# GuanRunwei/ASY-VRNet

Hardware: AMD Instinct MI355X
Metric: images/sec fwd+bwd, 512x512 img+4ch radar, bs=8/GPU (higher is better)
Workload: dtype f32; 1 GPU; EfficientVRNet(phi=l) forward+backward, 512x512 image + 4x512x512 radar, bs=8/GPU, fp32, det+seg heads (BASELINE.json configs[1]); random weights; global_batch=8, image_size=512, parallelism=dp1, launch=hipgraph

## Files before the change

### asy-vrnet_amd/csrc/fusion.hip

```cpp
#include "common.h"

namespace {

__device__ __forceinline__ f32x4 ld4(const float* p) { return *reinterpret_cast<const f32x4*>(p); }
__device__ __forceinline__ float bn_pre(float A, float x, float S, float D) { return __builtin_fmaf(A, x - S, D); }

__device__ __forceinline__ void col_stats_flush(const double (&s1)[4], const double (&s2)[4], int CV, double* partial, double* lds) {
  const int tid = threadIdx.x;
#pragma unroll
  for (int j = 0; j < 4; ++j) {
    lds[tid * 8 + j] = s1[j];
    lds[tid * 8 + 4 + j] = s2[j];
  }
  __syncthreads();
  if (tid < CV) {
    const int off = (int)(((long)blockIdx.x * 256) % CV);
    int t0 = tid - off;
    if (t0 < 0) t0 += CV;
    double a[4] = {0, 0, 0, 0}, b[4] = {0, 0, 0, 0};
    for (int t = t0; t < 256; t += CV)
#pragma unroll
      for (int j = 0; j < 4; ++j) {
        a[j] += lds[t * 8 + j];
        b[j] += lds[t * 8 + 4 + j];
      }
    double* o = partial + ((long)blockIdx.x * CV + tid) * 8;
#pragma unroll
    for (int j = 0; j < 4; ++j) {
      o[2 * j] = a[j];
      o[2 * j + 1] = b[j];
    }
  }
}

__device__ __forceinline__ void minmax_fold(const float* partial, int nblocks, float* smn, float* smx, float& mn, float& mx) {
  mn = INFINITY;
  mx = -INFINITY;
  for (int e = threadIdx.x; e < nblocks; e += 256) {
    mn = fminf(mn, partial[2 * e]);
    mx = fmaxf(mx, partial[2 * e + 1]);
  }
#pragma unroll
  for (int o = 32; o > 0; o >>= 1) {
    mn = fminf(mn, __shfl_xor(mn, o, 64));
    mx = fmaxf(mx, __shfl_xor(mx, o, 64));
  }
  if ((threadIdx.x & 63) == 0) {
    smn[threadIdx.x >> 6] = mn;
    smx[threadIdx.x >> 6] = mx;
  }
  __syncthreads();
  mn = fminf(fminf(smn[0], smn[1]), fminf(smn[2], smn[3]));
  mx = fmaxf(fmaxf(smx[0], smx[1]), fmaxf(smx[2], smx[3]));
}

template <bool RES>
__global__ __launch_bounds__(256) void bn_relu_kernel(const float* __restrict__ z, const float* __restrict__ A, const float* __restrict__ D,
                                                      const float* __restrict__ S, const float* __restrict__ res, float* __restrict__ out,
                                                      long n4, int C, float* __restrict__ mmpart, double* __restrict__ colpart) {
  __shared__ double lds[RES ? 256 * 8 : 1];
  __shared__ float smn[4], smx[4];
  const int CV = C >> 2;
  const long G = (long)gridDim.x * 256, e0 = (long)blockIdx.x * 256 + threadIdx.x;
  const int c0 = (int)(e0 % CV) * 4;
  const f32x4 a4 = ld4(A + c0), d4 = ld4(D + c0), s4 = ld4(S + c0);
  double s1[4] = {0, 0, 0, 0}, s2[4] = {0, 0, 0, 0};
  float mn = INFINITY, mx = -INFINITY;
  for (long e = e0; e < n4; e += G) {
    const f32x4 zv = ld4(z + 4 * e);
    f32x4 r4 = {0.f, 0.f, 0.f, 0.f}, o;
    if (RES) r4 = ld4(res + 4 * e);
#pragma unroll
    for (int j = 0; j < 4; ++j) {
      float v = fmaxf(bn_pre(a4[j], zv[j], s4[j], d4[j]), 0.f);
      if (RES) {
        v += r4[j];
        s1[j] += (double)v;
        s2[j] += (double)v * (double)v;
      } else {
        mn = fminf(mn, v);
        mx = fmaxf(mx, v);
      }
      o[j] = v;
    }
    *reinterpret_cast<f32x4*>(out + 4 * e) = o;
  }
  if (RES) {
    col_stats_flush(s1, s2, CV, colpart, lds);
  } else {
#pragma unroll
    for (int o = 32; o > 0; o >>= 1) {
      mn = fminf(mn, __shfl_xor(mn, o, 64));
      mx = fmaxf(mx, __shfl_xor(mx, o, 64));
    }
    if ((threadIdx.x & 63) == 0) {
      smn[threadIdx.x >> 6] = mn;
      smx[threadIdx.x >> 6] = mx;
    }
    __syncthreads();
    if (threadIdx.x == 0) {
      mmpart[2 * blockIdx.x] = fminf(fminf(smn[0], smn[1]), fminf(smn[2], smn[3]));
      mmpart[2 * blockIdx.x + 1] = fmaxf(fmaxf(smx[0], smx[1]), fmaxf(smx[2], smx[3]));
    }
  }
}

__global__ __launch_bounds__(256) void enhance_stats_kernel(const float* p, const float* x, const float* mmpart, int nmm, float* mm,
                                                            float* t, long n4, int C, double* colpart) {
  __shared__ double lds[256 * 8];
  __shared__ float smn[4], smx[4];
  float mn, mx;
  minmax_fold(mmpart, nmm, smn, smx, mn, mx);
  if (blockIdx.x == 0 && threadIdx.x == 0) { mm[0] = mn; mm[1] = mx; }
  const float dst = mx - mn;
  const int CV = C >> 2;
  const long G = (long)gridDim.x * 256, e0 = (long)blockIdx.x * 256 + threadIdx.x;
  double s1[4] = {0, 0, 0, 0}, s2[4] = {0, 0, 0, 0};
  for (long e = e0; e < n4; e += G) {
    const f32x4 pv = ld4(p + 4 * e), xv = ld4(x + 4 * e);
    f32x4 o;
#pragma unroll
    for (int j = 0; j < 4; ++j) {
      o[j] = (1.f + (pv[j] - mn) / dst) * xv[j];
      s1[j] += (double)o[j];
      s2[j] += (double)o[j] * (double)o[j];
    }
    *reinterpret_cast<f32x4*>(t + 4 * e) = o;
  }
  col_stats_flush(s1, s2, CV, colpart, lds);
}

__global__ __launch_bounds__(256) void bn_bwd_enhance_kernel(const float* g, const float* t, const float* A, const float* E,
                                                             const float* D, const float* S, const float* x, const float* p,
                                                             const float* mm, float* dt, long n4, int C, double* sums4) {
  __shared__ double red[4][4];
  const int CV = C >> 2;
  const long G = (long)gridDim.x * 256, e0 = (long)blockIdx.x * 256 + threadIdx.x;
  const int c0 = (int)(e0 % CV) * 4;
  const f32x4 a4 = ld4(A + c0), e4 = ld4(E + c0), d4 = ld4(D + c0), s4 = ld4(S + c0);
  const float mn = mm[0], mx = mm[1];
  double s[4] = {0, 0, 0, 0};
  for (long e = e0; e < n4; e += G) {
    const f32x4 gv = ld4(g + 4 * e), tv = ld4(t + 4 * e), xv = ld4(x + 4 * e), pv = ld4(p + 4 * e);
    f32x4 o;
#pragma unroll
    for (int j = 0; j < 4; ++j) {
      float v = a4[j] * gv[j];
      v += e4[j] * (tv[j] - s4[j]);
      v += d4[j];
      o[j] = v;
      const double dn = (double)v * (double)xv[j];
      s[0] += dn;
      s[1] += dn * (double)(pv[j] - mn);
      s[2] += (pv[j] == mn) ? 1.0 : 0.0;
      s[3] += (pv[j] == mx) ? 1.0 : 0.0;
    }
    *reinterpret_cast<f32x4*>(dt + 4 * e) = o;
  }
#pragma unroll
  for (int i = 0; i < 4; ++i) s[i] = wave_sum(s[i]);
  if ((threadIdx.x & 63) == 0)
#pragma unroll
    for (int i = 0; i < 4; ++i) red[threadIdx.x >> 6][i] = s[i];
  __syncthreads();
  if (threadIdx.x < 4)
    sums4[4 * (long)blockIdx.x + threadIdx.x] = red[0][threadIdx.x] + red[1][threadIdx.x] + red[2][threadIdx.x] + red[3][threadIdx.x];
}

__global__ __launch_bounds__(256) void enhance_bwd_stats_kernel(const float* dt, const float* x, const float* p, const float* mm,
                                                                const double* sums4, int nsums, const float* z, const float* fA,
                                                                const float* fD, const float* fS, float* dx, float* dp, long n4,
                                                                int C, int accumulate_dx, double* colpart) {
  __shared__ double lds[256 * 8];
  __shared__ double red[4][4];
  __shared__ double sums[4];
  {
    double s[4] = {0, 0, 0, 0};
    for (int e = threadIdx.x; e < nsums; e += 256)
#pragma unroll
      for (int i = 0; i < 4; ++i) s[i] += sums4[4 * (long)e + i];
#pragma unroll
    for (int i = 0; i < 4; ++i) s[i] = wave_sum(s[i]);
    if ((threadIdx.x & 63) == 0)
#pragma unroll
      for (int i = 0; i < 4; ++i) red[threadIdx.x >> 6][i] = s[i];
    __syncthreads();
    if (threadIdx.x < 4) sums[threadIdx.x] = red[0][threadIdx.x] + red[1][threadIdx.x] + red[2][threadIdx.x] + red[3][threadIdx.x];
    __syncthreads();
  }
  const float mn = mm[0], mx = mm[1];
  const double dstd = (double)mx - (double)mn;
  const float gmn = (float)((-sums[0] / dstd + sums[1] / (dstd * dstd)) / sums[2]);
  const float gmx = (float)((-sums[1] / (dstd * dstd)) / sums[3]);
  const float fd = (float)dstd;
  const int CV = C >> 2;
  const long G = (long)gridDim.x * 256, e0 = (long)blockIdx.x * 256 + threadIdx.x;
  const int c0 = (int)(e0 % CV) * 4;
  const f32x4 a4 = ld4(fA + c0), d4 = ld4(fD + c0), s4 = ld4(fS + c0);
  double s1[4] = {0, 0, 0, 0}, s2[4] = {0, 0, 0, 0};
  for (long e = e0; e < n4; e += G) {
    const f32x4 gv = ld4(dt + 4 * e), xv = ld4(x + 4 * e), pv = ld4(p + 4 * e), zv = ld4(z + 4 * e);
    f32x4 ox, op;
    if (accumulate_dx) ox = ld4(dx + 4 * e);
#pragma unroll
    for (int j = 0; j < 4; ++j) {
      const float gain = 1.f + (pv[j] - mn) / fd;
      const float vx = gv[j] * gain;
      ox[j] = accumulate_dx ? ox[j] + vx : vx;
      float v = gv[j] * xv[j] / fd;
      if (pv[j] == mn) v += gmn;
      if (pv[j] == mx) v += gmx;
      op[j] = v;
      const float vm = (bn_pre(a4[j], zv[j], s4[j], d4[j]) > 0.f) ? v : 0.f;
      s1[j] += (double)vm;
      s2[j] += (double)vm * (double)zv[j];
    }
    *reinterpret_cast<f32x4*>(dx + 4 * e) = ox;
    *reinterpret_cast<f32x4*>(dp + 4 * e) = op;
  }
  col_stats_flush(s1, s2, CV, colpart, lds);
}

__global__ __launch_bounds__(256) void bn_bwd_next_stats_kernel(const float* __restrict__ g, const float* __restrict__ sx,
                                                                const float* __restrict__ A, const float* __restrict__ E,
                                                                const float* __restrict__ D, const float* __restrict__ S,
                                                                const float* __restrict__ z, const float* __restrict__ fA,
                                                                const float* __restrict__ fD, const float* __restrict__ fS,
                                                                float* __restrict__ ds, long n4, int C, double* __restrict__ colpart) {
  __shared__ double lds[256 * 8];
  const int CV = C >> 2;
  const long G = (long)gridDim.x * 256, e0 = (long)blockIdx.x * 256 + threadIdx.x;
  const int c0 = (int)(e0 % CV) * 4;
  const f32x4 a4 = ld4(A + c0), e4 = ld4(E + c0), d4 = ld4(D + c0), s4 = ld4(S + c0);
  const f32x4 fa4 = ld4(fA + c0), fd4 = ld4(fD + c0), fs4 = ld4(fS + c0);
  double s1[4] = {0, 0, 0, 0}, s2[4] = {0, 0, 0, 0};
  for (long e = e0; e < n4; e += G) {
    const f32x4 gv = ld4(g + 4 * e), xv = ld4(sx + 4 * e), zv = ld4(z + 4 * e);
    f32x4 o;
#pragma unroll
    for (int j = 0; j < 4; ++j) {
      float v = a4[j] * gv[j];
      v += e4[j] * (xv[j] - s4[j]);
      v += d4[j];
      o[j] = v;
      const float vm = (bn_pre(fa4[j], zv[j], fs4[j], fd4[j]) > 0.f) ? v : 0.f;
      s1[j] += (double)vm;
      s2[j] += (double)vm * (double)zv[j];
    }
    *reinterpret_cast<f32x4*>(ds + 4 * e) = o;
  }
  col_stats_flush(s1, s2, CV, colpart, lds);
}

int fusion_grid(long n4, int CV, long cap = 4096) {
  int g = 256, a = CV;
  while (a) { const int t = g % a; g = a; a = t; }
  const int m = CV / g;
  long nb = vr_cdiv(n4, 256 * 2);
  if (nb > cap) nb = cap;
  if (nb < 1) nb = 1;
  nb = vr_cdiv(nb, m) * m;
  return (int)nb;
}
bool fusion_ok(long n, int C) { return C % 4 == 0 && C >= 4 && C <= 1024 && n % C == 0 && n / 4 < (1L << 40); }
#define FUSION_ALIGNED(...)                                                        \
  [&] {                                                                            \
    const void* ps_[] = {__VA_ARGS__};                                             \
    for (const void* q_ : ps_)                                                     \
      if (q_ && !vr_aligned16(q_)) return false;                                   \
    return true;                                                                   \
  }()

}

extern "C" int vrnet_fusion_chunks(long n, int C) { return fusion_ok(n, C) ? fusion_grid(n / 4, C / 4) : 0; }
extern "C" int vrnet_fusion_fold_chunks(long n, int C) { return fusion_ok(n, C) ? fusion_grid(n / 4, C / 4, 1024) : 0; }

extern "C" int vrnet_bn_relu_minmax_f32(const float* z, const float* A, const float* D, const float* S, float* p, long n, int C,
                                        float* mmpart, void* stream) {
  VR_CHECK_ARG(z && A && D && S && p && mmpart && fusion_ok(n, C) && FUSION_ALIGNED(z, A, D, S, p), "bn_relu_minmax: bad arguments");
  if (vr_ablated("affine")) return VR_OK;
  hipLaunchKernelGGL((bn_relu_kernel<false>), dim3(fusion_grid(n / 4, C / 4, 1024)), dim3(256), 0, vr_stream(stream), z, A, D, S,
                     (const float*)nullptr, p, n / 4, C, mmpart, (double*)nullptr);
  VR_LAUNCH_CHECK("bn_relu_minmax");
  return VR_OK;
}

extern "C" int vrnet_bn_relu_res_stats_f32(const float* z, const float* A, const float* D, const float* S, const float* res,
                                           float* s, long n, int C, double* colpart, void* stream) {
  VR_CHECK_ARG(z && A && D && S && res && s && colpart && fusion_ok(n, C) && FUSION_ALIGNED(z, A, D, S, res, s),
               "bn_relu_res_stats: bad arguments");
  if (vr_ablated("affine")) return VR_OK;
  hipLaunchKernelGGL((bn_relu_kernel<true>), dim3(fusion_grid(n / 4, C / 4)), dim3(256), 0, vr_stream(stream), z, A, D, S, res, s,
                     n / 4, C, (float*)nullptr, colpart);
  VR_LAUNCH_CHECK("bn_relu_res_stats");
  return VR_OK;
}

extern "C" int vrnet_enhance_stats_f32(const float* p, const float* x, const float* mmpart, int nmm, float* mm, float* t, long n,
                                       int C, double* colpart, void* stream) {
  VR_CHECK_ARG(p && x && mmpart && nmm > 0 && mm && t && colpart && fusion_ok(n, C) && FUSION_ALIGNED(p, x, t),
               "enhance_stats: bad arguments");
  if (vr_ablated("misc")) return VR_OK;
  hipLaunchKernelGGL(enhance_stats_kernel, dim3(fusion_grid(n / 4, C / 4)), dim3(256), 0, vr_stream(stream), p, x, mmpart, nmm, mm,
                     t, n / 4, C, colpart);
  VR_LAUNCH_CHECK("enhance_stats");
  return VR_OK;
}

extern "C" int vrnet_bn_bwd_enhance_f32(const float* g, const float* t, const float* A, const float* E, const float* D,
                                        const float* S, const float* x, const float* p, const float* mm, float* dt, long n, int C,
                                        double* sums4, void* stream) {
  VR_CHECK_ARG(g && t && A && E && D && S && x && p && mm && dt && sums4 && fusion_ok(n, C) &&
                   FUSION_ALIGNED(g, t, A, E, D, S, x, p, dt), "bn_bwd_enhance: bad arguments");
  if (vr_ablated("affine")) return VR_OK;
  hipLaunchKernelGGL(bn_bwd_enhance_kernel, dim3(fusion_grid(n / 4, C / 4, 1024)), dim3(256), 0, vr_stream(stream), g, t, A, E, D, S, x, p,
                     mm, dt, n / 4, C, sums4);
  VR_LAUNCH_CHECK("bn_bwd_enhance");
  return VR_OK;
}

extern "C" int vrnet_enhance_bwd_stats_f32(const float* dt, const float* x, const float* p, const float* mm, const double* sums4,
                                           int nsums, const float* z, const float* fA, const float* fD, const float* fS, float* dx,
                                           float* dp, long n, int C, int accumulate_dx, double* colpart, void* stream) {
  VR_CHECK_ARG(dt && x && p && mm && sums4 && nsums > 0 && z && fA && fD && fS && dx && dp && colpart && fusion_ok(n, C) &&
                   FUSION_ALIGNED(dt, x, p, z, fA, fD, fS, dx, dp), "enhance_bwd_stats: bad arguments");
  if (vr_ablated("misc")) return VR_OK;
  hipLaunchKernelGGL(enhance_bwd_stats_kernel, dim3(fusion_grid(n / 4, C / 4)), dim3(256), 0, vr_stream(stream), dt, x, p, mm, sums4,
                     nsums, z, fA, fD, fS, dx, dp, n / 4, C, accumulate_dx, colpart);
  VR_LAUNCH_CHECK("enhance_bwd_stats");
  return VR_OK;
}

extern "C" int vrnet_bn_bwd_next_stats_f32(const float* g, const float* s, const float* A, const float* E, const float* D,
                                           const float* S, const float* z, const float* fA, const float* fD, const float* fS,
                                           float* ds, long n, int C, double* colpart, void* stream) {
  VR_CHECK_ARG(g && s && A && E && D && S && z && fA && fD && fS && ds && colpart && fusion_ok(n, C) &&
                   FUSION_ALIGNED(g, s, A, E, D, S, z, fA, fD, fS, ds), "bn_bwd_next_stats: bad arguments");
  if (vr_ablated("affine")) return VR_OK;
  hipLaunchKernelGGL(bn_bwd_next_stats_kernel, dim3(fusion_grid(n / 4, C / 4)), dim3(256), 0, vr_stream(stream), g, s, A, E, D, S, z,
                     fA, fD, fS, ds, n / 4, C, colpart);
  VR_LAUNCH_CHECK("bn_bwd_next_stats");
  return VR_OK;
}
```

### asy-vrnet_amd/csrc/spatial.hip

```cpp
#include "common.h"

#include <cstdlib>

namespace {

__global__ __launch_bounds__(256) void dwconv3x3_kernel(const float* x, long ldx, const float* w, float* y, long ldy,
                                                        int B, int H, int W, int C, int flip, int accumulate) {
  const int total = B * H * W * C;
  for (int e = blockIdx.x * 256 + threadIdx.x; e < total; e += gridDim.x * 256) {
    const int c = e % C;
    const int pix = e / C;
    const int xx = pix % W;
    const int q = pix / W;
    const int yy = q % H;
    const int b = q / H;
    float s = 0.f;
#pragma unroll
    for (int ky = 0; ky < 3; ++ky) {
      const int sy = yy + ky - 1;
      if (sy < 0 || sy >= H) continue;
      const float* row = x + ((long)(b * H + sy) * W) * ldx + c;
#pragma unroll
      for (int kx = 0; kx < 3; ++kx) {
        const int sx = xx + kx - 1;
// ... 213 lines not shown
#pragma unroll
    for (int t = 0; t < 9; ++t) *reinterpret_cast<f32x4*>(smx + (((rest - 1) * quads + cq) * 9 + t) * 4) = acc[t];
  }
  __syncthreads();
  if (rest == 0 && c < C) {
    for (int r = 1; r < groups; ++r)
#pragma unroll
      for (int t = 0; t < 9; ++t) acc[t] += *reinterpret_cast<const f32x4*>(smx + (((r - 1) * quads + cq) * 9 + t) * 4);
    float* d = partial + ((long)blockIdx.x * C + c) * 9;
#pragma unroll
    for (int j = 0; j < 4; ++j)
#pragma unroll
      for (int t = 0; t < 9; ++t) d[j * 9 + t] = acc[t][j];
  }
}
__global__ __launch_bounds__(256) void dwconv3x3_wgrad_reduce_kernel(const float* partial, int nchunks, int C, float* dw,
                                                                     int accumulate) {
  __shared__ double red[16][16];
  const int o = threadIdx.x & 15, sl = threadIdx.x >> 4;
  const int e = blockIdx.x * 16 + o;
  const bool live = e < C * 9;
  double s = 0;
  if (live)
    for (int k = sl; k < nchunks; k += 16) s += partial[(long)k * C * 9 + e];
  red[sl][o] = s;
  __syncthreads();
  if (sl == 0 && live) {
#pragma unroll
    for (int k = 1; k < 16; ++k) s += red[k][o];
    dw[e] = (accumulate ? dw[e] : 0.f) + (float)s;
  }
}

__global__ __launch_bounds__(256) void patch_gather_kernel(const float* x, long ldx, const float* pos, float* out, int B,
                                                           int H, int W, int C, int CP, int k) {
  const int CT = C + CP, KT = k * k * CT, OH = H / k, OW = W / k;
  const long total = (long)B * OH * OW * KT;
  for (long e = (long)blockIdx.x * 256 + threadIdx.x; e < total; e += (long)gridDim.x * 256) {
    const int ch = e % KT;
    const long op = e / KT;
    const int t = ch / CT, c = ch - t * CT;
    const int ky = t / k, kx = t - ky * k;
    const int ox = op % OW;
    const long q = op / OW;
    const int oy = q % OH;
    const long b = q / OH;
    const int yy = oy * k + ky, xx = ox * k + kx;
    out[e] = c < C ? x[((b * H + yy) * W + xx) * ldx + c] : pos[((long)yy * W + xx) * CP + (c - C)];
  }
}
__global__ __launch_bounds__(256) void patch_scatter_kernel(const float* dp, float* dx, long lddx, int B, int H, int W, int C,
                                                            int CP, int k, int accumulate) {
  const int CT = C + CP, KT = k * k * CT, OH = H / k, OW = W / k;
  const long total = (long)B * H * W * C;
  for (long e = (long)blockIdx.x * 256 + threadIdx.x; e < total; e += (long)gridDim.x * 256) {
    const int c = e % C;
    const long pix = e / C;
    const int xx = pix % W;
    const long q = pix / W;
    const int yy = q % H;
    const long b = q / H;
    const int t = (yy % k) * k + (xx % k);
    const float v = dp[((b * OH + yy / k) * OW + xx / k) * KT + t * CT + c];
    float* d = dx + pix * lddx + c;
    *d = accumulate ? *d + v : v;
  }
}
__global__ void ohwi_kernel(const float* src, float* dst, int Cout, int Cin, int T, int dir, int accumulate) {
  const long total = (long)Cout * Cin * T;
  const long e = (long)blockIdx.x * blockDim.x + threadIdx.x;
  if (e >= total) return;
  const int t = e % T;
  const long q = e / T;
  const int c = q % Cin;
  const long n = q / Cin;
  const long oihw = e, ohwi = (n * T + t) * Cin + c;
  if (dir == 0) dst[ohwi] = src[oihw];
  else dst[oihw] = (accumulate ? dst[oihw] : 0.f) + src[ohwi];
}

template <bool FUSED_L = false>
__device__ __forceinline__ void src_index(float scale, int o, int in_size, int* i0, int* i1, float* l1) {
#pragma clang fp contract(off)
  const float r = scale * (float)o;
  int a = (int)r;
  if (a > in_size - 1) a = in_size - 1;
  *i0 = a;
  *i1 = a + ((a < in_size - 1) ? 1 : 0);
  *l1 = FUSED_L ? __builtin_fmaf(scale, (float)o, -(float)a) : r - (float)a;
}

__device__ __forceinline__ float up_tap(float v, bool bn, float a, float d, float s) {
  return bn ? fmaxf(__builtin_fmaf(a, v - s, d), 0.f) : v;
}
__device__ __forceinline__ float up_tap(float v, const float* bnA, const float* bnD, const float* bnS, int c) {
  return bnA ? up_tap(v, true, bnA[c], bnD[c], bnS[c]) : v;
}

// ... 1007 lines not shown
                                long workspace_bytes, void* stream) {
  if (vr_ablated("misc")) return VR_OK;
  VR_CHECK_ARG(dy && x && P && Q && Mn && mom && dx && EF && workspace, "sa_bwd: null tensor");
  VR_CHECK_ARG(workspace_bytes >= vrnet_sa_bwd_workspace(B, HW, C), "sa_bwd: workspace too small");
  int TPR, ncb, nchunks;
  long rows;
  sa_plan(HW, C, &TPR, &ncb, &nchunks, &rows);
  double* partial = reinterpret_cast<double*>(workspace);
  double* T = partial + (long)B * nchunks * C * 2;
  hipStream_t st = vr_stream(stream);
  hipLaunchKernelGGL(sa_bwd_reduce_kernel, dim3(nchunks, B, ncb), dim3(256), 256 * 2 * sizeof(double), st, dy, lddy, x,
                     ldx, P, Q, Mn, HW, C, TPR, rows, nchunks, partial);
  VR_LAUNCH_CHECK("sa_bwd_reduce");
  hipLaunchKernelGGL(sa_reduce_chunks_kernel, dim3(vr_cdiv((long)B * C * 2, 16)), dim3(256), 0, st, partial, T, B,
                     nchunks, C);
  VR_LAUNCH_CHECK("sa_reduce_chunks");
  SaParams sp{cw, cb, sw, sb, gnw, gnb};
  const int nb1 = (int)vr_cdiv((long)B * C, 256);
  float* E = EF;
  float* F = EF + (long)B * C;
  hipLaunchKernelGGL(sa_coef_bwd_kernel, dim3(nb1 + C / (2 * G)), dim3(256), 0, st, T, mom, sp, B, HW, C, G, nb1, E, F, dcw, dcb,
                     dsw, dsb, dgnw, dgnb, accumulate_params);
  VR_LAUNCH_CHECK("sa_coef_bwd");
  hipLaunchKernelGGL(sa_bwd_apply_kernel, dim3(grid_for(HW * C), B), dim3(256), 0, st, dy, lddy, x, ldx, P, Q, Mn, E, F, dx,
                     lddx, HW, C, accumulate_dx);
  VR_LAUNCH_CHECK("sa_bwd_apply");
  return VR_OK;
}

extern "C" int vrnet_patch_gather_f32(const float* x, long ldx, const float* pos, float* out, int B, int H, int W, int C,
                                      int CP, int k, void* stream) {
  VR_CHECK_ARG(x && out && (CP == 0 || pos) && B > 0 && C > 0 && CP >= 0 && k > 0 && H % k == 0 && W % k == 0 && ldx >= C,
               "patch_gather: bad arguments");
  hipLaunchKernelGGL(patch_gather_kernel, dim3(grid_for((long)B * H * W * (C + CP))), dim3(256), 0, vr_stream(stream), x,
                     ldx, pos, out, B, H, W, C, CP, k);
  VR_LAUNCH_CHECK("patch_gather");
  return VR_OK;
}

extern "C" int vrnet_patch_scatter_f32(const float* dp, float* dx, long lddx, int B, int H, int W, int C, int CP, int k,
                                       int accumulate, void* stream) {
  VR_CHECK_ARG(dp && dx && B > 0 && C > 0 && CP >= 0 && k > 0 && H % k == 0 && W % k == 0 && lddx >= C,
               "patch_scatter: bad arguments");
  hipLaunchKernelGGL(patch_scatter_kernel, dim3(grid_for((long)B * H * W * C)), dim3(256), 0, vr_stream(stream), dp, dx,
                     lddx, B, H, W, C, CP, k, accumulate);
  VR_LAUNCH_CHECK("patch_scatter");
  return VR_OK;
}

extern "C" int vrnet_weight_ohwi_f32(const float* src, float* dst, int Cout, int Cin, int kh, int kw, int dir,
                                     int accumulate, void* stream) {
  VR_CHECK_ARG(src && dst && Cout > 0 && Cin > 0 && kh > 0 && kw > 0 && (dir == 0 || dir == 1), "weight_ohwi: bad arguments");
  const long total = (long)Cout * Cin * kh * kw;
  hipLaunchKernelGGL(ohwi_kernel, dim3(vr_cdiv(total, 256)), dim3(256), 0, vr_stream(stream), src, dst, Cout, Cin, kh * kw,
                     dir, accumulate);
  VR_LAUNCH_CHECK("weight_ohwi");
  return VR_OK;
}
```

### asy-vrnet_amd/csrc/tinyconv.hip

```cpp
#include "common.h"

namespace tiny {

constexpr int CMAX = 8;

struct Args {
  const float* a; long lda; const float* w; const float* bias; float* y; long ldy;
  int B, H, W, Cin, Cout, k, pad, dil, accumulate;
};

template <int MODE>
__global__ __launch_bounds__(256) void conv_kernel(const Args p) {
  __shared__ float ws[9 * CMAX * CMAX];
  const int T = p.k * p.k;
  for (int i = threadIdx.x; i < T * p.Cout * p.Cin; i += 256) ws[i] = p.w[i];
  __syncthreads();
  const int CK = MODE == 0 ? p.Cin : p.Cout, CN = MODE == 0 ? p.Cout : p.Cin;
  const long total = (long)p.B * p.H * p.W;
  for (long pix = (long)blockIdx.x * 256 + threadIdx.x; pix < total; pix += (long)gridDim.x * 256) {
    const int x = pix % p.W;
    const long q = pix / p.W;
    const int y = q % p.H;
    const long b = q / p.H;
    float acc[CMAX];
// ... 216 lines not shown
    v += __builtin_bit_cast(float, __builtin_amdgcn_update_dpp(0, __builtin_bit_cast(int, v), 0x4E, 0xf, 0xf, true));
    v += __builtin_bit_cast(float, __builtin_amdgcn_update_dpp(0, __builtin_bit_cast(int, v), 0x141, 0xf, 0xf, true));
    v += __builtin_bit_cast(float, __builtin_amdgcn_update_dpp(0, __builtin_bit_cast(int, v), 0x140, 0xf, 0xf, true));
    return v;
  };
  const int rowid = threadIdx.x >> 4;
  const bool lead = (threadIdx.x & 15) == 0;
#pragma unroll
  for (int n = 0; n < NO; ++n) {
#pragma unroll
    for (int c = 0; c < CP; ++c)
#pragma unroll
      for (int t = 0; t < T; ++t) {
        const float sum = row16(acc[n][c][t]);
        if (lead) red[rowid][n * NA + c * T + t] = sum;
      }
    const float b = row16(bs[n]);
    if (lead) red[rowid][n * NA + CP * T] = b;
  }
  __syncthreads();
  const int per = Cin * T + 1;
  for (int i = threadIdx.x; i < NO * per; i += 256) {
    const int n = i / per, j = i - n * per;
    const int src = n * NA + (j == Cin * T ? CP * T : j);
    float sum = 0.f;
#pragma unroll
    for (int r = 0; r < 16; ++r) sum += red[r][src];
    partial[((long)blockIdx.x * NO + n) * per + j] = sum;
  }
}

__global__ __launch_bounds__(256) void wgrad_reduce_kernel(const float* partial, int nblk, int Cin, int Cout, int T,
                                                           const float* row_scale, float* dw, float* db, int accumulate) {
  __shared__ double red[16][16];
  const int per = Cin * T + 1;
  const int o = threadIdx.x & 15, sl = threadIdx.x >> 4;
  const int e = blockIdx.x * 16 + o;
  const bool live = e < Cout * per;
  const int n = live ? e / per : 0, i = e - n * per;
  double s = 0;
  if (live)
    for (int b = sl; b < nblk; b += 16) s += partial[((long)b * Cout + n) * per + i];
  red[sl][o] = s;
  __syncthreads();
  if (sl != 0 || !live) return;
#pragma unroll
  for (int k = 1; k < 16; ++k) s += red[k][o];
  float v = (float)s;
  if (row_scale) v *= row_scale[n];
  if (i == Cin * T) {
    if (db) db[n] = accumulate ? db[n] + v : v;
  } else {
    float* d = dw + (long)n * Cin * T + i;
    *d = accumulate ? *d + v : v;
  }
}

__global__ __launch_bounds__(256) void patch_dgrad_kernel(const float* dy, long lddy, const float* w, float* dx, long lddx,
                                                          int B, int H, int W, int Cin, int Cout, int k, int accumulate) {
  extern __shared__ float wsm[];
  const int T = k * k;
  for (int i = threadIdx.x; i < T * Cout * Cin; i += 256) wsm[i] = w[i];
  __syncthreads();
  const int OW = W / k, OH = H / k;
  const long total = (long)B * H * W;
  for (long pix = (long)blockIdx.x * 256 + threadIdx.x; pix < total; pix += (long)gridDim.x * 256) {
    const int x = pix % W;
    const long q = pix / W;
    const int y = q % H;
    const long b = q / H;
    const int t = (y % k) * k + (x % k);
    const float* g = dy + ((b * OH + y / k) * OW + x / k) * lddy;
    const float* wt = wsm + (long)t * Cout * Cin;
    float acc[CMAX];
#pragma unroll
    for (int c = 0; c < CMAX; ++c) acc[c] = 0.f;
    for (int n = 0; n < Cout; ++n) {
      const float gv = g[n];
#pragma unroll
      for (int c = 0; c < CMAX; ++c)
// ... 57 lines not shown
                  int B, int H, int W, int Cin, int Cout, int k, int pad, int dil, int accumulate, void* workspace,
                  hipStream_t st) {
  int nblk;
  long ppb;
  tiny_wgrad_plan((long)B * H * W, &nblk, &ppb);
  float* partial = reinterpret_cast<float*>(workspace);
  const int vec4 = Cin == 4 && ldx % 4 == 0 && vr_aligned16(x);
  dim3 grid(nblk, Cout), block(256);
#define VR_TINY_WGRAD_ALL(CP_, KS_, NO_)                                                                                 \
  do {                                                                                                                   \
    hipLaunchKernelGGL((tiny::wgrad_all_kernel<CP_, KS_, NO_>), dim3(nblk), block, 0, st, x, ldx, dy, lddy, B, H, W, Cin, pad, \
                       dil, vec4, ppb, partial);                                                                         \
    goto reduce;                                                                                                         \
  } while (0)
  if (k == 3 && Cin == 4 && Cout == 3) VR_TINY_WGRAD_ALL(4, 3, 3);
  if (k == 1 && Cin == 7 && Cout == 4) VR_TINY_WGRAD_ALL(8, 1, 4);
  if (k == 1 && Cin == 4 && Cout == 4) VR_TINY_WGRAD_ALL(4, 1, 4);
  if (k == 1 && Cin == 3 && Cout == 3) VR_TINY_WGRAD_ALL(4, 1, 3);
#undef VR_TINY_WGRAD_ALL
#define VR_TINY_WGRAD(CP_, KS_)                                                                                          \
  hipLaunchKernelGGL((tiny::wgrad_kernel<CP_, KS_>), grid, block, 0, st, x, ldx, dy, lddy, B, H, W, Cin, Cout, pad, dil, vec4, \
                     ppb, partial)
  if (k == 1) {
    if (Cin <= 4) VR_TINY_WGRAD(4, 1);
    else VR_TINY_WGRAD(8, 1);
  } else {
    if (Cin <= 4) VR_TINY_WGRAD(4, 3);
    else VR_TINY_WGRAD(8, 3);
  }
#undef VR_TINY_WGRAD
reduce:
  VR_LAUNCH_CHECK("tiny_wgrad");
  const int per = Cin * k * k + 1;
  hipLaunchKernelGGL(tiny::wgrad_reduce_kernel, dim3(vr_cdiv(Cout * per, 16)), dim3(256), 0, st, partial, nblk, Cin, Cout,
                     k * k, row_scale, dw, db, accumulate);
  VR_LAUNCH_CHECK("tiny_wgrad_reduce");
  return VR_OK;
}

int vr_patch_dgrad(const float* dy, long lddy, const float* w, float* dx, long lddx, int B, int H, int W, int Cin,
                   int Cout, int k, int accumulate, hipStream_t st) {
  long blocks = vr_cdiv((long)B * H * W, 256);
  if (blocks > 16384) blocks = 16384;
  const size_t lds = (size_t)k * k * Cout * Cin * sizeof(float);
  hipLaunchKernelGGL(tiny::patch_dgrad_kernel, dim3(blocks), dim3(256), lds, st, dy, lddy, w, dx, lddx, B, H, W, Cin, Cout,
                     k, accumulate);
  VR_LAUNCH_CHECK("patch_dgrad");
  return VR_OK;
}
```

Before: 339.2 images/sec.

## Extend fused BN kernels to narrow channels, vectorize patch gather/scatter, rework wgrad reduce

The fused BN/enhance kernels now accept channel counts that are not multiples of 4 (up to 32), using a period-based coefficient mapping and a per-channel fold of the column statistics. Small-channel tensors can then take the fused path instead of a slower fallback. Patch gather/scatter is restructured to one thread per output patch row, with templated vectorized variants for the (3,2,4) and (4,2,4) cases that replace the old per-element index math. The tiny wgrad reduce now uses one workgroup per output element with a wave shuffle reduction instead of 16-wide strided partial sums. The cost is extra complexity in the stats flush and more template instantiations.

```diff
diff --git a/asy-vrnet_amd/csrc/fusion.hip b/asy-vrnet_amd/csrc/fusion.hip
--- a/asy-vrnet_amd/csrc/fusion.hip
+++ b/asy-vrnet_amd/csrc/fusion.hip
@@ -5,14 +5,51 @@
 __device__ __forceinline__ f32x4 ld4(const float* p) { return *reinterpret_cast<const f32x4*>(p); }
 __device__ __forceinline__ float bn_pre(float A, float x, float S, float D) { return __builtin_fmaf(A, x - S, D); }
 
-__device__ __forceinline__ void col_stats_flush(const double (&s1)[4], const double (&s2)[4], int CV, double* partial, double* lds) {
-  const int tid = threadIdx.x;
+constexpr int NARROW_MAX_C = 32;
+__host__ __device__ __forceinline__ int fusion_period(int C) { return (C & 3) == 0 ? C >> 2 : ((C & 1) ? C : C >> 1); }
+__device__ __forceinline__ f32x4 ld_coef(const float* a, int q, int C) {
+  if ((C & 3) == 0) return ld4(a + 4 * q);
+  f32x4 v;
+#pragma unroll
+  for (int j = 0; j < 4; ++j) v[j] = a[(4 * q + j) % C];
+  return v;
+}
+
+__device__ __forceinline__ void col_stats_flush(const double (&s1)[4], const double (&s2)[4], int C, double* partial, double* lds) {
+  const int tid = threadIdx.x, CV = fusion_period(C);
 #pragma unroll
   for (int j = 0; j < 4; ++j) {
     lds[tid * 8 + j] = s1[j];
     lds[tid * 8 + 4 + j] = s2[j];
   }
   __syncthreads();
+  if (C & 3) {
+    __shared__ double part[4 * NARROW_MAX_C * 2];
+    if (tid < 4 * C) {
+      const int c = tid >> 2, j = tid & 3;
+      int q = -1;
+      for (int k = 0, ch = j % C; k < CV; ++k, ch = (ch + 4) % C)
+        if (ch == c) { q = k; break; }
+      double a = 0, b = 0;
+      if (q >= 0) {
+        int t0 = q - (int)(((long)blockIdx.x * 256) % CV);
+        if (t0 < 0) t0 += CV;
+        for (int t = t0; t < 256; t += CV) {
+          a += lds[t * 8 + j];
+          b += lds[t * 8 + 4 + j];
+        }
+      }
+      part[2 * tid] = a;
+      part[2 * tid + 1] = b;
+    }
+    __syncthreads();
+    if (tid < C) {
+      double* o = partial + ((long)blockIdx.x * C + tid) * 2;
+      o[0] = ((part[8 * tid] + part[8 * tid + 2]) + part[8 * tid + 4]) + part[8 * tid + 6];
+      o[1] = ((part[8 * tid + 1] + part[8 * tid + 3]) + part[8 * tid + 5]) + part[8 * tid + 7];
+    }
+    return;
+  }
   if (tid < CV) {
     const int off = (int)(((long)blockIdx.x * 256) % CV);
     int t0 = tid - off;
@@ -60,10 +97,10 @@
                                                       long n4, int C, float* __restrict__ mmpart, double* __restrict__ colpart) {
   __shared__ double lds[RES ? 256 * 8 : 1];
   __shared__ float smn[4], smx[4];
-  const int CV = C >> 2;
-  const long G = (long)gridDim.x * 256, e0 = (long)blockIdx.x * 256 + threadIdx.x;
-  const int c0 = (int)(e0 % CV) * 4;
-  const f32x4 a4 = ld4(A + c0), d4 = ld4(D + c0), s4 = ld4(S + c0);
+  const int CV = fusion_period(C);
+  const long G = (long)gridDim.x * 256, e0 = (long)blockIdx.x * 256 + threadIdx.x;
+  const int q0 = (int)(e0 % CV);
+  const f32x4 a4 = ld_coef(A, q0, C), d4 = ld_coef(D, q0, C), s4 = ld_coef(S, q0, C);
   double s1[4] = {0, 0, 0, 0}, s2[4] = {0, 0, 0, 0};
   float mn = INFINITY, mx = -INFINITY;
   for (long e = e0; e < n4; e += G) {
@@ -86,7 +123,7 @@
     *reinterpret_cast<f32x4*>(out + 4 * e) = o;
   }
   if (RES) {
-    col_stats_flush(s1, s2, CV, colpart, lds);
+    col_stats_flush(s1, s2, C, colpart, lds);
   } else {
 #pragma unroll
     for (int o = 32; o > 0; o >>= 1) {
@@ -113,7 +150,6 @@
   minmax_fold(mmpart, nmm, smn, smx, mn, mx);
   if (blockIdx.x == 0 && threadIdx.x == 0) { mm[0] = mn; mm[1] = mx; }
   const float dst = mx - mn;
-  const int CV = C >> 2;
   const long G = (long)gridDim.x * 256, e0 = (long)blockIdx.x * 256 + threadIdx.x;
   double s1[4] = {0, 0, 0, 0}, s2[4] = {0, 0, 0, 0};
   for (long e = e0; e < n4; e += G) {
@@ -127,17 +163,17 @@
     }
     *reinterpret_cast<f32x4*>(t + 4 * e) = o;
   }
-  col_stats_flush(s1, s2, CV, colpart, lds);
+  col_stats_flush(s1, s2, C, colpart, lds);
 }
 
 __global__ __launch_bounds__(256) void bn_bwd_enhance_kernel(const float* g, const float* t, const float* A, const float* E,
                                                              const float* D, const float* S, const float* x, const float* p,
                                                              const float* mm, float* dt, long n4, int C, double* sums4) {
   __shared__ double red[4][4];
-  const int CV = C >> 2;
-  const long G = (long)gridDim.x * 256, e0 = (long)blockIdx.x * 256 + threadIdx.x;
-  const int c0 = (int)(e0 % CV) * 4;
-  const f32x4 a4 = ld4(A + c0), e4 = ld4(E + c0), d4 = ld4(D + c0), s4 = ld4(S + c0);
+  const int CV = fusion_period(C);
+  const long G = (long)gridDim.x * 256, e0 = (long)blockIdx.x * 256 + threadIdx.x;
+  const int q0 = (int)(e0 % CV);
+  const f32x4 a4 = ld_coef(A, q0, C), e4 = ld_coef(E, q0, C), d4 = ld_coef(D, q0, C), s4 = ld_coef(S, q0, C);
   const float mn = mm[0], mx = mm[1];
   double s[4] = {0, 0, 0, 0};
   for (long e = e0; e < n4; e += G) {
@@ -193,10 +229,10 @@
   const float gmn = (float)((-sums[0] / dstd + sums[1] / (dstd * dstd)) / sums[2]);
   const float gmx = (float)((-sums[1] / (dstd * dstd)) / sums[3]);
   const float fd = (float)dstd;
-  const int CV = C >> 2;
-  const long G = (long)gridDim.x * 256, e0 = (long)blockIdx.x * 256 + threadIdx.x;
-  const int c0 = (int)(e0 % CV) * 4;
-  const f32x4 a4 = ld4(fA + c0), d4 = ld4(fD + c0), s4 = ld4(fS + c0);
+  const int CV = fusion_period(C);
+  const long G = (long)gridDim.x * 256, e0 = (long)blockIdx.x * 256 + threadIdx.x;
+  const int q0 = (int)(e0 % CV);
+  const f32x4 a4 = ld_coef(fA, q0, C), d4 = ld_coef(fD, q0, C), s4 = ld_coef(fS, q0, C);
   double s1[4] = {0, 0, 0, 0}, s2[4] = {0, 0, 0, 0};
   for (long e = e0; e < n4; e += G) {
     const f32x4 gv = ld4(dt + 4 * e), xv = ld4(x + 4 * e), pv = ld4(p + 4 * e), zv = ld4(z + 4 * e);
@@ -218,7 +254,7 @@
     *reinterpret_cast<f32x4*>(dx + 4 * e) = ox;
     *reinterpret_cast<f32x4*>(dp + 4 * e) = op;
   }
-  col_stats_flush(s1, s2, CV, colpart, lds);
+  col_stats_flush(s1, s2, C, colpart, lds);
 }
 
 __global__ __launch_bounds__(256) void bn_bwd_next_stats_kernel(const float* __restrict__ g, const float* __restrict__ sx,
@@ -228,11 +264,11 @@
                                                                 const float* __restrict__ fD, const float* __restrict__ fS,
                                                                 float* __restrict__ ds, long n4, int C, double* __restrict__ colpart) {
   __shared__ double lds[256 * 8];
-  const int CV = C >> 2;
-  const long G = (long)gridDim.x * 256, e0 = (long)blockIdx.x * 256 + threadIdx.x;
-  const int c0 = (int)(e0 % CV) * 4;
-  const f32x4 a4 = ld4(A + c0), e4 = ld4(E + c0), d4 = ld4(D + c0), s4 = ld4(S + c0);
-  const f32x4 fa4 = ld4(fA + c0), fd4 = ld4(fD + c0), fs4 = ld4(fS + c0);
+  const int CV = fusion_period(C);
+  const long G = (long)gridDim.x * 256, e0 = (long)blockIdx.x * 256 + threadIdx.x;
+  const int q0 = (int)(e0 % CV);
+  const f32x4 a4 = ld_coef(A, q0, C), e4 = ld_coef(E, q0, C), d4 = ld_coef(D, q0, C), s4 = ld_coef(S, q0, C);
+  const f32x4 fa4 = ld_coef(fA, q0, C), fd4 = ld_coef(fD, q0, C), fs4 = ld_coef(fS, q0, C);
   double s1[4] = {0, 0, 0, 0}, s2[4] = {0, 0, 0, 0};
   for (long e = e0; e < n4; e += G) {
     const f32x4 gv = ld4(g + 4 * e), xv = ld4(sx + 4 * e), zv = ld4(z + 4 * e);
@@ -249,7 +285,7 @@
     }
     *reinterpret_cast<f32x4*>(ds + 4 * e) = o;
   }
-  col_stats_flush(s1, s2, CV, colpart, lds);
+  col_stats_flush(s1, s2, C, colpart, lds);
 }
 
 int fusion_grid(long n4, int CV, long cap = 4096) {
@@ -262,7 +298,10 @@
   nb = vr_cdiv(nb, m) * m;
   return (int)nb;
 }
-bool fusion_ok(long n, int C) { return C % 4 == 0 && C >= 4 && C <= 1024 && n % C == 0 && n / 4 < (1L << 40); }
+bool fusion_ok(long n, int C) {
+  const bool width = C % 4 == 0 ? (C >= 4 && C <= 1024) : (C >= 1 && C <= NARROW_MAX_C && n % 4 == 0);
+  return width && n % C == 0 && n / 4 < (1L << 40);
+}
 #define FUSION_ALIGNED(...)                                                        \
   [&] {                                                                            \
     const void* ps_[] = {__VA_ARGS__};                                             \
@@ -273,14 +312,14 @@
 
 }
 
-extern "C" int vrnet_fusion_chunks(long n, int C) { return fusion_ok(n, C) ? fusion_grid(n / 4, C / 4) : 0; }
-extern "C" int vrnet_fusion_fold_chunks(long n, int C) { return fusion_ok(n, C) ? fusion_grid(n / 4, C / 4, 1024) : 0; }
+extern "C" int vrnet_fusion_chunks(long n, int C) { return fusion_ok(n, C) ? fusion_grid(n / 4, fusion_period(C)) : 0; }
+extern "C" int vrnet_fusion_fold_chunks(long n, int C) { return fusion_ok(n, C) ? fusion_grid(n / 4, fusion_period(C), 1024) : 0; }
 
 extern "C" int vrnet_bn_relu_minmax_f32(const float* z, const float* A, const float* D, const float* S, float* p, long n, int C,
                                         float* mmpart, void* stream) {
   VR_CHECK_ARG(z && A && D && S && p && mmpart && fusion_ok(n, C) && FUSION_ALIGNED(z, A, D, S, p), "bn_relu_minmax: bad arguments");
   if (vr_ablated("affine")) return VR_OK;
-  hipLaunchKernelGGL((bn_relu_kernel<false>), dim3(fusion_grid(n / 4, C / 4, 1024)), dim3(256), 0, vr_stream(stream), z, A, D, S,
+  hipLaunchKernelGGL((bn_relu_kernel<false>), dim3(fusion_grid(n / 4, fusion_period(C), 1024)), dim3(256), 0, vr_stream(stream), z, A, D, S,
                      (const float*)nullptr, p, n / 4, C, mmpart, (double*)nullptr);
   VR_LAUNCH_CHECK("bn_relu_minmax");
   return VR_OK;
@@ -291,7 +330,7 @@
   VR_CHECK_ARG(z && A && D && S && res && s && colpart && fusion_ok(n, C) && FUSION_ALIGNED(z, A, D, S, res, s),
                "bn_relu_res_stats: bad arguments");
   if (vr_ablated("affine")) return VR_OK;
-  hipLaunchKernelGGL((bn_relu_kernel<true>), dim3(fusion_grid(n / 4, C / 4)), dim3(256), 0, vr_stream(stream), z, A, D, S, res, s,
+  hipLaunchKernelGGL((bn_relu_kernel<true>), dim3(fusion_grid(n / 4, fusion_period(C))), dim3(256), 0, vr_stream(stream), z, A, D, S, res, s,
                      n / 4, C, (float*)nullptr, colpart);
   VR_LAUNCH_CHECK("bn_relu_res_stats");
   return VR_OK;
@@ -302,7 +341,7 @@
   VR_CHECK_ARG(p && x && mmpart && nmm > 0 && mm && t && colpart && fusion_ok(n, C) && FUSION_ALIGNED(p, x, t),
                "enhance_stats: bad arguments");
   if (vr_ablated("misc")) return VR_OK;
-  hipLaunchKernelGGL(enhance_stats_kernel, dim3(fusion_grid(n / 4, C / 4)), dim3(256), 0, vr_stream(stream), p, x, mmpart, nmm, mm,
+  hipLaunchKernelGGL(enhance_stats_kernel, dim3(fusion_grid(n / 4, fusion_period(C))), dim3(256), 0, vr_stream(stream), p, x, mmpart, nmm, mm,
                      t, n / 4, C, colpart);
   VR_LAUNCH_CHECK("enhance_stats");
   return VR_OK;
@@ -314,7 +353,7 @@
   VR_CHECK_ARG(g && t && A && E && D && S && x && p && mm && dt && sums4 && fusion_ok(n, C) &&
                    FUSION_ALIGNED(g, t, A, E, D, S, x, p, dt), "bn_bwd_enhance: bad arguments");
   if (vr_ablated("affine")) return VR_OK;
-  hipLaunchKernelGGL(bn_bwd_enhance_kernel, dim3(fusion_grid(n / 4, C / 4, 1024)), dim3(256), 0, vr_stream(stream), g, t, A, E, D, S, x, p,
+  hipLaunchKernelGGL(bn_bwd_enhance_kernel, dim3(fusion_grid(n / 4, fusion_period(C), 1024)), dim3(256), 0, vr_stream(stream), g, t, A, E, D, S, x, p,
                      mm, dt, n / 4, C, sums4);
   VR_LAUNCH_CHECK("bn_bwd_enhance");
   return VR_OK;
@@ -326,7 +365,7 @@
   VR_CHECK_ARG(dt && x && p && mm && sums4 && nsums > 0 && z && fA && fD && fS && dx && dp && colpart && fusion_ok(n, C) &&
                    FUSION_ALIGNED(dt, x, p, z, fA, fD, fS, dx, dp), "enhance_bwd_stats: bad arguments");
   if (vr_ablated("misc")) return VR_OK;
-  hipLaunchKernelGGL(enhance_bwd_stats_kernel, dim3(fusion_grid(n / 4, C / 4)), dim3(256), 0, vr_stream(stream), dt, x, p, mm, sums4,
+  hipLaunchKernelGGL(enhance_bwd_stats_kernel, dim3(fusion_grid(n / 4, fusion_period(C))), dim3(256), 0, vr_stream(stream), dt, x, p, mm, sums4,
                      nsums, z, fA, fD, fS, dx, dp, n / 4, C, accumulate_dx, colpart);
   VR_LAUNCH_CHECK("enhance_bwd_stats");
   return VR_OK;
@@ -338,7 +377,7 @@
   VR_CHECK_ARG(g && s && A && E && D && S && z && fA && fD && fS && ds && colpart && fusion_ok(n, C) &&
                    FUSION_ALIGNED(g, s, A, E, D, S, z, fA, fD, fS, ds), "bn_bwd_next_stats: bad arguments");
   if (vr_ablated("affine")) return VR_OK;
-  hipLaunchKernelGGL(bn_bwd_next_stats_kernel, dim3(fusion_grid(n / 4, C / 4)), dim3(256), 0, vr_stream(stream), g, s, A, E, D, S, z,
+  hipLaunchKernelGGL(bn_bwd_next_stats_kernel, dim3(fusion_grid(n / 4, fusion_period(C))), dim3(256), 0, vr_stream(stream), g, s, A, E, D, S, z,
                      fA, fD, fS, ds, n / 4, C, colpart);
   VR_LAUNCH_CHECK("bn_bwd_next_stats");
   return VR_OK;
diff --git a/asy-vrnet_amd/csrc/spatial.hip b/asy-vrnet_amd/csrc/spatial.hip
--- a/asy-vrnet_amd/csrc/spatial.hip
+++ b/asy-vrnet_amd/csrc/spatial.hip
@@ -269,38 +269,127 @@
   }
 }
 
-__global__ __launch_bounds__(256) void patch_gather_kernel(const float* x, long ldx, const float* pos, float* out, int B,
-                                                           int H, int W, int C, int CP, int k) {
-  const int CT = C + CP, KT = k * k * CT, OH = H / k, OW = W / k;
-  const long total = (long)B * OH * OW * KT;
-  for (long e = (long)blockIdx.x * 256 + threadIdx.x; e < total; e += (long)gridDim.x * 256) {
-    const int ch = e % KT;
-    const long op = e / KT;
-    const int t = ch / CT, c = ch - t * CT;
-    const int ky = t / k, kx = t - ky * k;
-    const int ox = op % OW;
-    const long q = op / OW;
-    const int oy = q % OH;
-    const long b = q / OH;
-    const int yy = oy * k + ky, xx = ox * k + kx;
-    out[e] = c < C ? x[((b * H + yy) * W + xx) * ldx + c] : pos[((long)yy * W + xx) * CP + (c - C)];
-  }
-}
-__global__ __launch_bounds__(256) void patch_scatter_kernel(const float* dp, float* dx, long lddx, int B, int H, int W, int C,
-                                                            int CP, int k, int accumulate) {
-  const int CT = C + CP, KT = k * k * CT, OH = H / k, OW = W / k;
-  const long total = (long)B * H * W * C;
-  for (long e = (long)blockIdx.x * 256 + threadIdx.x; e < total; e += (long)gridDim.x * 256) {
-    const int c = e % C;
-    const long pix = e / C;
-    const int xx = pix % W;
-    const long q = pix / W;
-    const int yy = q % H;
-    const long b = q / H;
-    const int t = (yy % k) * k + (xx % k);
-    const float v = dp[((b * OH + yy / k) * OW + xx / k) * KT + t * CT + c];
-    float* d = dx + pix * lddx + c;
-    *d = accumulate ? *d + v : v;
+struct PatchRow {
+  unsigned b, yy, ox, e;
+  long drow;
+  bool live;
+};
+__device__ __forceinline__ PatchRow patch_row(int H, int W, int k, int segs) {
+  const unsigned OH = (unsigned)(H / k), WK = (unsigned)(W / k) * (unsigned)k;
+  const unsigned row = blockIdx.x / (unsigned)segs;
+  PatchRow p;
+  p.e = (blockIdx.x - row * (unsigned)segs) * 256u + threadIdx.x;
+  p.live = p.e < WK;
+  p.b = row / OH;
+  p.ox = p.e / (unsigned)k;
+  p.yy = (row - p.b * OH) * (unsigned)k + (p.e - p.ox * (unsigned)k);
+  p.drow = (long)row * WK + p.e;
+  return p;
+}
+
+__global__ __launch_bounds__(256) void patch_gather_kernel(const float* x, long ldx, const float* pos, float* out, int H, int W,
+                                                           int C, int CP, int k, int segs) {
+  const PatchRow p = patch_row(H, W, k, segs);
+  if (!p.live) return;
+  const float* xs = x + (((long)p.b * H + p.yy) * W + (long)p.ox * k) * ldx;
+  const float* ps = pos + ((long)p.yy * W + (long)p.ox * k) * CP;
+  float* d = out + p.drow * (k * (C + CP));
+  for (int kx = 0; kx < k; ++kx) {
+    for (int c = 0; c < C; ++c) *d++ = xs[kx * ldx + c];
+    for (int c = 0; c < CP; ++c) *d++ = ps[kx * CP + c];
+  }
+}
+template <int C, int CP, int K, bool XV>
+__global__ __launch_bounds__(256) void patch_gather_vec_kernel(const float* x, long ldx, const float* pos, float* out, int H,
+                                                               int W, int segs) {
+  constexpr int CT = C + CP;
+  static_assert((K * C) % 4 == 0 && (K * CP) % 4 == 0, "patch rows in 16-byte words");
+  const PatchRow p = patch_row(H, W, K, segs);
+  if (!p.live) return;
+  const float* xs = x + (((long)p.b * H + p.yy) * W + (long)p.ox * K) * ldx;
+  float xv[K * C], pv[K * CP + 1], v[K * CT];
+  if (XV) {
+#pragma unroll
+    for (int q = 0; q < K * C / 4; ++q) {
+      const f32x4 t = reinterpret_cast<const f32x4*>(xs)[q];
+#pragma unroll
+      for (int j = 0; j < 4; ++j) xv[4 * q + j] = t[j];
+    }
+  } else {
+#pragma unroll
+    for (int kx = 0; kx < K; ++kx)
+#pragma unroll
+      for (int c = 0; c < C; ++c) xv[kx * C + c] = xs[kx * ldx + c];
+  }
+  if (CP > 0) {
+    const f32x4* ps = reinterpret_cast<const f32x4*>(pos + ((long)p.yy * W + (long)p.ox * K) * CP);
+#pragma unroll
+    for (int q = 0; q < K * CP / 4; ++q) {
+      const f32x4 t = ps[q];
+#pragma unroll
+      for (int j = 0; j < 4; ++j) pv[4 * q + j] = t[j];
+    }
+  }
+#pragma unroll
+  for (int kx = 0; kx < K; ++kx) {
+#pragma unroll
+    for (int c = 0; c < C; ++c) v[kx * CT + c] = xv[kx * C + c];
+#pragma unroll
+    for (int c = 0; c < CP; ++c) v[kx * CT + C + c] = pv[kx * CP + c];
+  }
+  f32x4* d = reinterpret_cast<f32x4*>(out + p.drow * (K * CT));
+#pragma unroll
+  for (int q = 0; q < K * CT / 4; ++q) d[q] = f32x4{v[4 * q], v[4 * q + 1], v[4 * q + 2], v[4 * q + 3]};
+}
+__global__ __launch_bounds__(256) void patch_scatter_kernel(const float* dp, float* dx, long lddx, int H, int W, int C, int CP,
+                                                            int k, int segs, int accumulate) {
+  const PatchRow p = patch_row(H, W, k, segs);
+  if (!p.live) return;
+  const float* s = dp + p.drow * (k * (C + CP));
+  float* d = dx + (((long)p.b * H + p.yy) * W + (long)p.ox * k) * lddx;
+  for (int kx = 0; kx < k; ++kx)
+    for (int c = 0; c < C; ++c) {
+      const float v = s[kx * (C + CP) + c];
+      float* o = d + kx * lddx + c;
+      *o = accumulate ? *o + v : v;
+    }
+}
+template <int C, int CP, int K, bool XV>
+__global__ __launch_bounds__(256) void patch_scatter_vec_kernel(const float* dp, float* dx, long lddx, int H, int W, int segs,
+                                                                int accumulate) {
+  constexpr int CT = C + CP;
+  static_assert((K * C) % 4 == 0 && (K * CP) % 4 == 0, "patch rows in 16-byte words");
+  const PatchRow p = patch_row(H, W, K, segs);
+  if (!p.live) return;
+  const f32x4* s = reinterpret_cast<const f32x4*>(dp + p.drow * (K * CT));
+  float v[K * CT], xv[K * C];
+#pragma unroll
+  for (int q = 0; q < K * CT / 4; ++q) {
+    const f32x4 t = s[q];
+#pragma unroll
+    for (int j = 0; j < 4; ++j) v[4 * q + j] = t[j];
+  }
+#pragma unroll
+  for (int kx = 0; kx < K; ++kx)
+#pragma unroll
+    for (int c = 0; c < C; ++c) xv[kx * C + c] = v[kx * CT + c];
+  float* d = dx + (((long)p.b * H + p.yy) * W + (long)p.ox * K) * lddx;
+  if (XV) {
+    f32x4* d4 = reinterpret_cast<f32x4*>(d);
+#pragma unroll
+    for (int q = 0; q < K * C / 4; ++q) {
+      f32x4 t{xv[4 * q], xv[4 * q + 1], xv[4 * q + 2], xv[4 * q + 3]};
+      if (accumulate) t = d4[q] + t;
+      d4[q] = t;
+    }
+  } else {
+#pragma unroll
+    for (int kx = 0; kx < K; ++kx)
+#pragma unroll
+      for (int c = 0; c < C; ++c) {
+        float* o = d + kx * lddx + c;
+        *o = accumulate ? *o + xv[kx * C + c] : xv[kx * C + c];
+      }
   }
 }
 __global__ void ohwi_kernel(const float* src, float* dst, int Cout, int Cin, int T, int dir, int accumulate) {
@@ -1374,8 +1463,25 @@
                                       int CP, int k, void* stream) {
   VR_CHECK_ARG(x && out && (CP == 0 || pos) && B > 0 && C > 0 && CP >= 0 && k > 0 && H % k == 0 && W % k == 0 && ldx >= C,
                "patch_gather: bad arguments");
-  hipLaunchKernelGGL(patch_gather_kernel, dim3(grid_for((long)B * H * W * (C + CP))), dim3(256), 0, vr_stream(stream), x,
-                     ldx, pos, out, B, H, W, C, CP, k);
+  const int segs = (int)vr_cdiv(W, 256);
+  const long nwg = (long)B * (H / k) * segs;
+  VR_CHECK_ARG(nwg < (1L << 31), "patch_gather: too many output rows for one launch");
+  hipStream_t st = vr_stream(stream);
+  const bool al = vr_aligned16(out) && (CP == 0 || vr_aligned16(pos));
+  const bool xv = ldx == C && vr_aligned16(x);
+#define VR_PATCH_GATHER(C_, CP_, K_)                                                                                     \
+  if (al && C == C_ && CP == CP_ && k == K_) {                                                                           \
+    if (xv) hipLaunchKernelGGL((patch_gather_vec_kernel<C_, CP_, K_, true>), dim3(nwg), dim3(256), 0, st, x, ldx, pos, out, H, \
+                               W, segs);                                                                                 \
+    else hipLaunchKernelGGL((patch_gather_vec_kernel<C_, CP_, K_, false>), dim3(nwg), dim3(256), 0, st, x, ldx, pos, out, H,  \
+                            W, segs);                                                                                    \
+    VR_LAUNCH_CHECK("patch_gather");                                                                                     \
+    return VR_OK;                                                                                                        \
+  }
+  VR_PATCH_GATHER(3, 2, 4)
+  VR_PATCH_GATHER(4, 2, 4)
+#undef VR_PATCH_GATHER
+  hipLaunchKernelGGL(patch_gather_kernel, dim3(nwg), dim3(256), 0, st, x, ldx, pos, out, H, W, C, CP, k, segs);
   VR_LAUNCH_CHECK("patch_gather");
   return VR_OK;
 }
@@ -1384,8 +1490,25 @@
                                        int accumulate, void* stream) {
   VR_CHECK_ARG(dp && dx && B > 0 && C > 0 && CP >= 0 && k > 0 && H % k == 0 && W % k == 0 && lddx >= C,
                "patch_scatter: bad arguments");
-  hipLaunchKernelGGL(patch_scatter_kernel, dim3(grid_for((long)B * H * W * C)), dim3(256), 0, vr_stream(stream), dp, dx,
-                     lddx, B, H, W, C, CP, k, accumulate);
+  const int segs = (int)vr_cdiv(W, 256);
+  const long nwg = (long)B * (H / k) * segs;
+  VR_CHECK_ARG(nwg < (1L << 31), "patch_scatter: too many output rows for one launch");
+  hipStream_t st = vr_stream(stream);
+  const bool al = vr_aligned16(dp);
+  const bool xv = lddx == C && vr_aligned16(dx);
+#define VR_PATCH_SCATTER(C_, CP_, K_)                                                                                    \
+  if (al && C == C_ && CP == CP_ && k == K_) {                                                                           \
+    if (xv) hipLaunchKernelGGL((patch_scatter_vec_kernel<C_, CP_, K_, true>), dim3(nwg), dim3(256), 0, st, dp, dx, lddx, H, W, \
+                               segs, accumulate);                                                                        \
+    else hipLaunchKernelGGL((patch_scatter_vec_kernel<C_, CP_, K_, false>), dim3(nwg), dim3(256), 0, st, dp, dx, lddx, H, W,  \
+                            segs, accumulate);                                                                           \
+    VR_LAUNCH_CHECK("patch_scatter");                                                                                    \
+    return VR_OK;                                                                                                        \
+  }
+  VR_PATCH_SCATTER(3, 2, 4)
+  VR_PATCH_SCATTER(4, 2, 4)
+#undef VR_PATCH_SCATTER
+  hipLaunchKernelGGL(patch_scatter_kernel, dim3(nwg), dim3(256), 0, st, dp, dx, lddx, H, W, C, CP, k, segs, accumulate);
   VR_LAUNCH_CHECK("patch_scatter");
   return VR_OK;
 }
diff --git a/asy-vrnet_amd/csrc/tinyconv.hip b/asy-vrnet_amd/csrc/tinyconv.hip
--- a/asy-vrnet_amd/csrc/tinyconv.hip
+++ b/asy-vrnet_amd/csrc/tinyconv.hip
@@ -272,20 +272,25 @@
 
 __global__ __launch_bounds__(256) void wgrad_reduce_kernel(const float* partial, int nblk, int Cin, int Cout, int T,
                                                            const float* row_scale, float* dw, float* db, int accumulate) {
-  __shared__ double red[16][16];
+  __shared__ double red[4];
   const int per = Cin * T + 1;
-  const int o = threadIdx.x & 15, sl = threadIdx.x >> 4;
-  const int e = blockIdx.x * 16 + o;
-  const bool live = e < Cout * per;
-  const int n = live ? e / per : 0, i = e - n * per;
+  const int e = blockIdx.x;
+  const int n = e / per, i = e - n * per;
+  const long stride = (long)Cout * per;
+  const float* src = partial + e;
   double s = 0;
-  if (live)
-    for (int b = sl; b < nblk; b += 16) s += partial[((long)b * Cout + n) * per + i];
-  red[sl][o] = s;
-  __syncthreads();
-  if (sl != 0 || !live) return;
-#pragma unroll
-  for (int k = 1; k < 16; ++k) s += red[k][o];
+  int b = threadIdx.x;
+  for (; b + 768 < nblk; b += 1024) {
+    const float v0 = src[b * stride], v1 = src[(b + 256) * stride], v2 = src[(b + 512) * stride], v3 = src[(b + 768) * stride];
+    s += v0; s += v1; s += v2; s += v3;
+  }
+  for (; b < nblk; b += 256) s += src[b * stride];
+#pragma unroll
+  for (int m = 1; m < 64; m <<= 1) s += __shfl_xor(s, m);
+  if ((threadIdx.x & 63) == 0) red[threadIdx.x >> 6] = s;
+  __syncthreads();
+  if (threadIdx.x != 0) return;
+  s = ((red[0] + red[1]) + red[2]) + red[3];
   float v = (float)s;
   if (row_scale) v *= row_scale[n];
   if (i == Cin * T) {
@@ -409,7 +414,7 @@
 reduce:
   VR_LAUNCH_CHECK("tiny_wgrad");
   const int per = Cin * k * k + 1;
-  hipLaunchKernelGGL(tiny::wgrad_reduce_kernel, dim3(vr_cdiv(Cout * per, 16)), dim3(256), 0, st, partial, nblk, Cin, Cout,
+  hipLaunchKernelGGL(tiny::wgrad_reduce_kernel, dim3(Cout * per), dim3(256), 0, st, partial, nblk, Cin, Cout,
                      k * k, row_scale, dw, db, accumulate);
   VR_LAUNCH_CHECK("tiny_wgrad_reduce");
   return VR_OK;
```

Result: no change. 339.9 images/sec, median of 6 (+0.2%).
